# jgsimard/RustRobotics

Measured on AMD Instinct MI355X. Metric: GN iterations/s, higher is better.
Workload: dtype f64; 1 GPU; intel (1728 poses / 4830 edges / dim 5184), Gauss-Newton, one graph on one GPU; solver=GaussNewton, parallelism=single

## Files before the change

### rustrobotics_amd/csrc/kernels.hip.h

```cpp
#pragma once
#include <hip/hip_runtime.h>

#include <cstdint>
#include <type_traits>

#ifndef RRPGO_CHAIN_PRIO
#define RRPGO_CHAIN_PRIO 3
#endif

namespace rrpgo {

constexpr unsigned X_PENDING_WORD = 0x7ff8deadu;

template <typename T> struct VecT;
template <> struct VecT<float> { using V4 = float4; using V2 = float2; };
template <> struct VecT<double> { using V4 = double4; using V2 = double2; };

#ifndef RRPGO_LIN_GROUP
#define RRPGO_LIN_GROUP 8
#endif
constexpr int LIN_GROUP = RRPGO_LIN_GROUP;
constexpr int LIN_THREADS = 256;
constexpr int UPD_THREADS = 256;

// ... 41 lines not shown
#endif
#else
#define RRPGO_STAMP(a, s, slot) do { } while (0)
#define RRPGO_STAMP_SOLVE(a, s, slot) do { } while (0)
#define RRPGO_ACC_DECL() do { } while (0)
#define RRPGO_ACC_BEGIN() do { } while (0)
#define RRPGO_ACC_END(ptr, slot) do { } while (0)
#endif

__device__ __forceinline__ int wave_index() { return __builtin_amdgcn_readfirstlane((int)(threadIdx.x >> 6)); }

enum : int { DEVERR_NOT_SPD = 1, DEVERR_FLOW_TIMEOUT = 2 };

struct OptCtrl {
  double lambda;
  double last_error;
  double tolerance;
  unsigned long long seq;
  int reject;
  int pad;
};
struct alignas(32) OptSlot {
  double chi2, norm;
  int flags, pad;
  unsigned long long seq;
};
enum : int { OPT_RING = 8 };
enum : int { OPT_STOP = 1,
             OPT_SKIPPED = 2,
             OPT_ERR_SHIFT = 8
};
__device__ __forceinline__ void opt_publish(OptCtrl *c, OptSlot *ring, double chi2, double norm, int flags) {
  const unsigned long long n = c->seq + 1;
  OptSlot *s = ring + (n - 1) % OPT_RING;
  s->chi2 = chi2;
  s->norm = norm;
  s->flags = flags;
  __hip_atomic_store(&s->seq, n, __ATOMIC_RELEASE, __HIP_MEMORY_SCOPE_SYSTEM);
  c->seq = n;
}
__device__ __forceinline__ bool opt_stopped(const int *err) { return err && err[1] != 0; }


template <typename TC> struct EdgeRec {
  int32_t from, to;
  int64_t slot;
  typename VecT<TC>::V4 meas;
  typename VecT<TC>::V4 info_a;
  typename VecT<TC>::V2 info_b;
};
static_assert(sizeof(EdgeRec<float>) == 64 && sizeof(EdgeRec<double>) == 128, "EdgeRec is four / eight sixteen-byte loads of one line");
template <typename T, typename TC = T> struct LinArgs {
  int n_nodes;
  const EdgeRec<TC> *e_rec;
  const typename VecT<TC>::V4 *pose;
  const int2 *e_idx;
  const typename VecT<TC>::V4 *e_meas;
  const typename VecT<TC>::V4 *e_info_a;
  const typename VecT<TC>::V2 *e_info_b;
// ... 198 lines not shown

template <typename A> __device__ __forceinline__ void opt_publish_chi2_in_last_block(const A &a, double *red) {
  if (!a.publish) return;
  const bool stopped = !a.reset_ctrl && a.err[1] != 0;
  if (a.publish == 1 && !stopped) return;
  __shared__ int is_last;
  if (threadIdx.x == 0) {
    __threadfence();
    is_last = atomicAdd(a.blocks_done, 1) == (int)gridDim.x - 1;
  }
  __syncthreads();
  if (!is_last) return;
  __threadfence();
  double c = 0.0;
  for (int i = threadIdx.x; i < (int)gridDim.x; i += LIN_THREADS) c += a.chi2_partial[i];
  const double ct = block_sum<double, LIN_THREADS>(c, red);
  if (threadIdx.x == 0) {
    *a.blocks_done = 0;
    if (!stopped) a.ctrl->last_error = ct;
    opt_publish(a.ctrl, a.ring_host, ct, 0.0, stopped ? OPT_SKIPPED : 0);
  }
}

template <typename TO, typename T, int RK = ROBUST_NONE>
__global__ void __launch_bounds__(LIN_THREADS) k_linearize(LinArgs<TO, T> a) {
  using V4 = typename VecT<T>::V4;
  using V2 = typename VecT<T>::V2;
  __shared__ double red[LIN_THREADS / 64];
  const int gid = blockIdx.x * LIN_THREADS + threadIdx.x;
  for (int i = gid; i < a.n_zero_words; i += gridDim.x * LIN_THREADS) a.zero_words[i] = 0u;
  for (int i = gid; i < a.n_fill_words; i += gridDim.x * LIN_THREADS) a.fill_words[i] = X_PENDING_WORD;
  opt_reset_in_first_thread(a);
  const T lambda = a.lambda_from_ctrl ? (T)a.ctrl->lambda : a.lambda;
  const int slot = gid / LIN_GROUP, sub = gid % LIN_GROUP;
  const int node = slot < a.n_nodes ? (a.node_list ? a.node_list[slot] : slot) : -1;
  double chi = 0.0;
  T hd[6] = {0, 0, 0, 0, 0, 0};
  T bv[3] = {0, 0, 0};
  int nd = 0;
  if (node >= 0) {
    nd = a.node_dim[node];
    const V4 self = a.pose[node];
    const int q1 = a.inc_ptr[node + 1];
    for (int q = a.inc_ptr[node] + sub; q < q1; q += LIN_GROUP) {
      const int2 inc = a.inc_list[q];
      const int ent = inc.x;
      if (!(ent & 12)) continue;
      const bool owns = ent & 4;
      const int k = ent >> 4, kind = (ent >> 1) & 1, role = ent & 1;
      const EdgeRec<T> rec = a.e_rec[k];
      const V4 other = a.pose[inc.y];
      const V4 z = rec.meas;
      const V4 wa = rec.info_a;
      const V2 wb = rec.info_b;
      T W[3][3] = {{wa.x, wa.y, wa.z}, {wa.y, wa.w, wb.x}, {wa.z, wb.x, wb.y}};
      T e[3], A[3][3], B[3][3];
      edge_linearize_2d<T>(kind, role ? other : self, role ? self : other, z, e, A, B);
      T s_rob = 0;
      bool rob = false;
      if constexpr (RK != ROBUST_NONE) {
        s_rob = edge_chi2_2d<T>(W, e);
        rob = !a.robust_mask || a.robust_mask[k];
        if (rob) {
          const T w = robust_weight<RK, T>(s_rob, a.robust_delta, a.robust_delta2);
#pragma unroll
          for (int i = 0; i < 3; i++)
#pragma unroll
            for (int j = 0; j < 3; j++) W[i][j] *= w;
        }
      }
      T JW[3][3];
#pragma unroll
      for (int i = 0; i < 3; i++)
#pragma unroll
// ... 43 lines not shown
  if (a.write_system) {
#pragma unroll
    for (int t = 0; t < 6; t++) hd[t] = group_sum8(hd[t]);
#pragma unroll
    for (int t = 0; t < 3; t++) bv[t] = group_sum8(bv[t]);
    if (node >= 0 && sub == 0) {
      T add = lambda;
      if (node == a.anchor) add += (T)10000000.0;
      if (a.adds_diag && !a.adds_diag[node]) add = 0;
      TO *d = a.hvals + a.diag_off[node];
      if (nd == 3) {
        d[0] = (TO)(hd[0] + add); d[1] = (TO)hd[1];         d[2] = (TO)hd[3];
        d[3] = (TO)hd[1];         d[4] = (TO)(hd[2] + add); d[5] = (TO)hd[4];
        d[6] = (TO)hd[3];         d[7] = (TO)hd[4];         d[8] = (TO)(hd[5] + add);
      } else {
        d[0] = (TO)(hd[0] + add); d[1] = (TO)hd[1];
        d[2] = (TO)hd[1];         d[3] = (TO)(hd[2] + add);
      }
      TO *bo = a.b + a.node_offset[node];
      for (int t = 0; t < nd; t++) bo[t] = (TO)(-bv[t]);
    }
  }
  double tot = block_sum<double, LIN_THREADS>(chi, red);
  if (threadIdx.x == 0) a.chi2_partial[blockIdx.x] = tot;
  opt_publish_chi2_in_last_block(a, red);
}

template <typename TO, typename T>
__global__ void __launch_bounds__(256) k_lin_init(LinArgs<TO, T> a) {
  const int node = blockIdx.x * 256 + threadIdx.x;
  if (node >= a.n_nodes) return;
  const int nd = a.node_dim[node];
  T add = a.lambda;
  if (node == a.anchor) add += (T)10000000.0;
  TO *d = a.hvals + a.diag_off[node];
  for (int t = 0; t < nd * nd; t++) d[t] = (t / nd == t % nd) ? (TO)add : (TO)0;
  TO *bo = a.b + a.node_offset[node];
  for (int t = 0; t < nd; t++) bo[t] = 0;
}
template <typename TO, typename T>
__global__ void __launch_bounds__(256) k_lin_finish(LinArgs<TO, T> a) {
  const int node = blockIdx.x * 256 + threadIdx.x;
  if (node >= a.n_nodes) return;
  const int nd = a.node_dim[node];
  TO *d = a.hvals + a.diag_off[node];
  for (int i = 0; i < nd; i++)
    for (int j = i + 1; j < nd; j++) d[i * nd + j] = d[j * nd + i];
// ... 3005 lines not shown
  for (int i = j + threadIdx.x; i < a.nc; i += 256) col[i] += a0 * v0[i] + a1 * v1[i] + a2 * v2[i];
}


template <typename T, typename TC = T> struct UpdArgs {
  int n_nodes;
  typename VecT<TC>::V4 *pose;
  const uint8_t *node_dim;
  const int32_t *node_pcol, *node_offset;
  const T *x;
  const T *dx_ref_in;
  T *dx_ref_out;
  TC sign;
  double *norm_partial;
  int gauge_anchor;
  int export_only;
  const int *err;
  const int32_t *node_list;
  const uint8_t *norm_counts;
  const int *gate;
  FinArgs fin;
};

template <typename TO, typename T>
__device__ __forceinline__ double update_node(const UpdArgs<TO, T> &a, int node) {
  double nrm = 0.0;
  const int nd = a.node_dim[node];
  T d[3] = {0, 0, 0};
  const TO *src = a.dx_ref_in ? a.dx_ref_in + a.node_offset[node] : a.x + a.node_pcol[node];
  for (int t = 0; t < nd; t++) d[t] = (T)src[t];
  auto p = a.pose[node];
  const bool regauge = a.gauge_anchor >= 0 && !a.dx_ref_in;
  if (regauge) {
    const TO *ya = a.x + a.node_pcol[a.gauge_anchor];
    const T c0 = (T)ya[0], c1 = (T)ya[1], c2 = (T)ya[2];
    const auto pa = a.pose[a.gauge_anchor];
    d[0] = d[0] - c0 + c2 * (p.y - pa.y);
    d[1] = d[1] - c1 - c2 * (p.x - pa.x);
    if (nd == 3) d[2] -= c2;
    if (node == a.gauge_anchor) { d[0] = 0; d[1] = 0; d[2] = 0; }
  }
  if (a.dx_ref_out) {
    TO *dst = a.dx_ref_out + a.node_offset[node];
    for (int t = 0; t < nd; t++) dst[t] = (TO)d[t];
  }
  if (!a.export_only && !(regauge && node == a.gauge_anchor)) {
    if (!a.norm_counts || a.norm_counts[node])
      for (int t = 0; t < nd; t++) nrm += (double)d[t] * (double)d[t];
    p.x += a.sign * d[0];
    p.y += a.sign * d[1];
    if (nd == 3) {
      const T c = cos(a.sign * d[2]), s = sin(a.sign * d[2]);
      const T re = p.z * c - p.w * s, im = p.z * s + p.w * c;
      p.z = re;
      p.w = im;
    }
    a.pose[node] = p;
  }
  return nrm;
}

template <typename TO, typename T>
__global__ void __launch_bounds__(UPD_THREADS) k_update(UpdArgs<TO, T> a) {
  __shared__ double red[UPD_THREADS / 64];
  const int slot = blockIdx.x * UPD_THREADS + threadIdx.x;
  const int node = slot < a.n_nodes ? (a.node_list ? a.node_list[slot] : slot) : -1;
  double nrm = 0.0;
  if (a.gate && *a.gate == 0) return;
  const bool failed = a.err && (a.err[0] != 0 || a.err[1] != 0);
  if (node >= 0 && !failed) nrm = update_node(a, node);
  if (a.export_only) return;
  double tot = block_sum<double, UPD_THREADS>(nrm, red);
  if (threadIdx.x == 0) a.norm_partial[blockIdx.x] = tot;
  if (a.fin.enabled) finalize_in_last_block<UPD_THREADS>(a.fin, a.norm_partial, (int)gridDim.x, red);
}

}
```

### rustrobotics_amd/csrc/lds_flow.hip.h

```cpp
#pragma once

namespace rrpgo {

struct alignas(128) LdsFlowTask {
  SnMeta m;
  int32_t sn;
  int32_t sn_begin, sn_end;
  int32_t kind;
  int32_t slices;
  int32_t bx, by;
  int32_t n_units;
  int32_t pad[8];
};
static_assert(sizeof(LdsFlowTask) == 128, "LdsFlowTask is one 128-byte line");

__device__ __forceinline__ int lds_flow_ticket(unsigned *ticket, int *slot) {
  if (threadIdx.x == 0) *slot = (int)atomicAdd(ticket, 1u);
  __syncthreads();
  return __builtin_amdgcn_readfirstlane(*slot);
}

template <typename T, int THREADS>
__global__ void __launch_bounds__(THREADS) k_factor_flow(FactorArgs<T> a, const LdsFlowTask *tasks, int n_tasks, unsigned *ticket) {
  extern __shared__ __align__(16) unsigned char smem_raw[];
// ... 59 lines not shown
      __syncthreads();
      if (threadIdx.x == 0) __hip_atomic_fetch_add(a.dep_flags + a.parent_dep_self + tr.sn, 1u, __ATOMIC_RELAXED, __HIP_MEMORY_SCOPE_AGENT);
      continue;
    }
    if (tr.kind == 2) {
      dep_wait_count(a.dep_flags + a.parent_dep_self + tr.sn, (unsigned)tr.n_units, a.err, a.wait_ticks);
      solve_big_front<T, THREADS, true>(a, tr.m, smem, part, N, tr.slices);
      continue;
    }
    int snext = tr.sn;
    SnMeta mnext = tr.m;
    for (int si = tr.sn_end - 1; si >= tr.sn_begin; si--) {
      const int s = snext;
      const SnMeta m = mnext;
      if (si > tr.sn_begin) {
        snext = a.task_sn[si - 1];
        mnext = a.sn_meta[snext];
      }
      solve_front<T, THREADS, true, true>(a, s, m, smem);
    }
  }
}

__global__ void __launch_bounds__(256) k_fill_words(unsigned *w, int n, unsigned v) {
  for (int i = blockIdx.x * 256 + threadIdx.x; i < n; i += gridDim.x * 256) w[i] = v;
}

__global__ void __launch_bounds__(256) k_copy_words16(const uint4 *src, uint4 *dst, int64_t n) {
  for (int64_t i = (int64_t)blockIdx.x * 256 + threadIdx.x; i < n; i += (int64_t)gridDim.x * 256) dst[i] = src[i];
}

}
```

### rustrobotics_amd/csrc/pgo_api.hip

```cpp
#include <mutex>
#include <queue>
#include <hip/hip_runtime.h>

#include <algorithm>
#include <chrono>
#include <cmath>
#include <cstdio>
#include <cstdlib>
#include <cstring>
#include <functional>
#include <memory>
#include <stdexcept>
#include <string>
#include <thread>
#include <vector>

#include "../../include/rr_pgo.h"
#include "host_graph.h"
#include "kernels.hip.h"
#include "flow.hip.h"
#include "lds_flow.hip.h"
#include "selinv.hip.h"
#include "treesolve.hip.h"
#include "symbolic.h"
// ... 367 lines not shown
  static constexpr int kGemvSlices = 16;
  DevBuf<double> chi_partial_, norm_partial_, hist_;
  DevBuf<int> counter_, err_, blocks_done_;
  DevBuf<unsigned long long> stamps_;
  DevBuf<int32_t> task_ptr_, task_sn_, fasm_src_, fasm_dst_, fasm_colptr_, fdup_src_, fdup_dst_, scat_, rel_, perm_, sn_rows_;
  DevBuf<SnMeta> sn_meta_, task_meta_;
  DevBuf<ChildMeta> child_meta_;
  std::vector<int> step_solve_lds_;
  PinnedBuf<double> host_pair_;
  PinnedBuf<V4> state_stage_;
  EventHolder state_stage_ev_;
  std::vector<double> state_in_;
  DevBuf<V4> pose_saved_;
  OptSlot *opt_ring_ = nullptr;
  DevBuf<OptCtrl> opt_ctrl_;
  bool opt_active_ = false;
  bool opt_first_ = false;
  bool opt_lambda_dev_ = false;
  int opt_publish_ = 0;
  double opt_lambda0_ = 0.01;
  bool stop_dirty_ = false;
  bool sync_optimize_ = false;
  int n_lin_blocks_ = 0, n_upd_blocks_ = 0;
  bool no_graph_ = false, force_graph_ = false;
  bool edge_lin_ = false;
  bool edge_lin_wave_ = false;
  bool edge_lin_env_ = false, edge_lin_wave_env_ = false;
  int lin_blocks_pull_ = 0, lin_blocks_edge_ = 0;
  int robust_kind_ = ROBUST_NONE;
  double robust_delta_ = 1.0;
  DevBuf<uint8_t> robust_mask_;
  int host_counter_ = 0;

 public:
  Engine(const HostGraph &g, const Symbolic &sym, int rank, int world, bool sharded)
      : g_(g), sym_(sym), rank_(rank), world_(world), sharded_(sharded || world > 1) {
    struct ArenaScope {
      explicit ArenaScope(DeviceArena *a) { t_arena = a; }
      ~ArenaScope() { t_arena = nullptr; }
    } scope(&arena_);
    const bool ctimes = getenv("RR_PGO_ANALYZE_TIMES") != nullptr;
    double ct0 = now_ms();
    auto cmark = [&](const char *what) {
      if (!ctimes) return;
      const double t = now_ms();
      std::fprintf(stderr, "engine:  %-12s %8.3f ms\n", what, t - ct0);
// ... 137 lines not shown
      bool any_big = false;
      for (const Step &st : sym.steps) any_big = any_big || st.kind != STEP_TASKS;
      gemv_part_.alloc(any_big ? (size_t)kGemvSlices * g.dim : 4);
    }
    if (const char *e = getenv("RR_PGO_SOLVE_THREADS")) solve_threads_max_ = std::atoi(e);
    if (const char *e = getenv("RR_PGO_SP_SOLVE_MIN")) sp_solve_min_nc_ = std::atoi(e);
    if (const char *e = getenv("RR_PGO_SCHUR_SPLIT")) schur_split_ = std::atoi(e) != 0;
    no_graph_ = getenv("RR_PGO_NO_GRAPH") != nullptr;
    force_graph_ = getenv("RR_PGO_FORCE_GRAPH") != nullptr && !no_graph_;
    if (const char *e = getenv("RR_PGO_FLOW")) flow_max_nf_ = std::atoi(e);
    if (const char *e = getenv("RR_PGO_FLOW_EXACT")) flow_exact_ = std::atoi(e) != 0;
    if (const char *e = getenv("RR_PGO_FLOW_TASKS")) flow_max_tasks_ = std::atoi(e);
    if (const char *e = getenv("RR_PGO_SOLVE_FLOW")) solve_flow_on_ = std::atoi(e) != 0;
    if (const char *e = getenv("RR_PGO_FLOW_SCHUR_MIN")) flow_schur_min_ = std::atoi(e);
    n_lin_blocks_ = (int)(((int64_t)n_list_ * LIN_GROUP + LIN_THREADS - 1) / LIN_THREADS);
    lin_blocks_pull_ = n_lin_blocks_;
    edge_lin_ = getenv("RR_PGO_EDGE_LINEARIZE") != nullptr && !is3d_ && !sharded_ && g_.n_edges() > 0;
    edge_lin_wave_ = edge_lin_ && std::atoi(getenv("RR_PGO_EDGE_LINEARIZE")) == 2;
    if (edge_lin_) n_lin_blocks_ = std::max(1, (g_.n_edges() + (edge_lin_wave_ ? WE_EDGES : LIN_THREADS) - 1) / (edge_lin_wave_ ? WE_EDGES : LIN_THREADS));
    edge_lin_env_ = edge_lin_;
    edge_lin_wave_env_ = edge_lin_wave_;
    lin_blocks_edge_ = n_lin_blocks_;
    n_upd_blocks_ = (n_list_ + UPD_THREADS - 1) / UPD_THREADS;
    chi_partial_.alloc((size_t)(edge_lin_ ? std::max(lin_blocks_pull_, lin_blocks_edge_) : n_lin_blocks_));
    norm_partial_.alloc((size_t)n_upd_blocks_);
    hist_.alloc(2 * HIST);
    hist_.zero();
    counter_.alloc(1);
    counter_.zero();
    err_.alloc(2);
    err_.zero();
    opt_ctrl_.alloc(1);
    opt_ctrl_.zero();
    sync_optimize_ = getenv("RR_PGO_SYNC_OPTIMIZE") != nullptr;
    blocks_done_.alloc(2);
    blocks_done_.zero();
    cmark("numeric");
    task_ptr_.upload(sym.task_ptr);
    task_sn_.upload(sym.task_sn);
    {
      std::vector<SnMeta> meta(sym.S);
      std::vector<ChildMeta> cm(sym.child_list.size());
      int64_t wblk_total = 0;
      for (int f = 0; f < sym.S; f++) {
        SnMeta &m = meta[f];
        m.nc = sym.sn_ncols[f];
        m.nr = sym.sn_nrows[f];
// ... 151 lines not shown
        for (int t = st.task_begin; t < st.task_end; t++) {
          int s = sym.task_sn[sym.task_ptr[t]];
          need = std::max(need, sym.sn_ncols[s] + sym.sn_nrows[s] + 64 * 65 + 4);
        }
      }
      if ((size_t)need * sizeof(T) > (size_t)kMaxLds) throw ApiError(RR_PGO_EUNSUPPORTED, "front too large for the back-substitution scratch");
      step_solve_lds_.push_back(need);
    }
#ifdef RRPGO_STAMPS
    stamps_.alloc((size_t)sym.S * 12 + 400000);
    stamps_.zero();
#endif
    plan_mid_solve_tasks();
    cmark("index tables");
    configure_kernels();
    cmark("kernel attrs");
    n_launches_per_iter = 2;
    for (const Step &st : sym.steps)
      n_launches_per_iter += st.kind == STEP_BIG ? count_big_launches(st) + count_big_solve_launches(st) : 2;
    if (lds_flow_) {
      n_launches_per_iter = 4 + (xl_ ? 1 : 0);
      for (size_t si = 1; si < sym.steps.size(); si++)
        n_launches_per_iter += (xl_ ? 0 : count_big_launches(sym.steps[si])) + (mid_in_flow_[si] ? 0 : count_big_solve_launches(sym.steps[si]));
    }
  }

  ~Engine() override {
    if (gn_exec_) (void)hipGraphExecDestroy(gn_exec_);
    for (hipGraphExec_t e : stage_exec_) if (e) (void)hipGraphExecDestroy(e);
  }

  hipStream_t stream() override { return stream_; }

 private:
  void build_flow_levels() {
    flow_levels_.clear();
    flow_levels_.resize(sym_.steps.size());
    solve_flow_.clear();
    solve_flow_.resize(sym_.steps.size());
    constexpr double kDiag = 4.0, kPre = 2.5, kNewest = 1.5, kX = 1.5, kLook = 4.5, kTile = 8.0, kTail = 4.5, kHop = 0.7;
    int64_t words = 0;
    int dev = 0, cus = 256;
    HIPCHK(hipGetDevice(&dev));
    (void)hipDeviceGetAttribute(&cus, hipDeviceAttributeMultiprocessorCount, dev);
    flow_grid_ = std::max(cus, 1) * (sizeof(T) == 4 ? RRPGO_FLOW_WAVES : 1);
    if (const char *e = getenv("RR_PGO_FLOW_GRID")) flow_grid_ = std::max(1, std::atoi(e));
// ... 703 lines not shown
    int64_t n[RR_PGO_NUM_KCLASS] = {0};
  } prof_;
  void pbegin() { if (prof_.on) HIPCHK(hipEventRecord(prof_.e0, stream_)); }
  void pend(int k, int launches = 1) {
    if (!prof_.on) return;
    HIPCHK(hipEventRecord(prof_.e1, stream_));
    HIPCHK(hipEventSynchronize(prof_.e1));
    float ms = 0;
    HIPCHK(hipEventElapsedTime(&ms, prof_.e0, prof_.e1));
    prof_.ms[k] += ms;
    prof_.n[k] += launches;
  }

  void check_launch(const char *what) {
    hipError_t e = hipGetLastError();
    if (e != hipSuccess) throw ApiError(RR_PGO_ENODEVICE, std::string("kernel launch failed (") + what + "): " + hipGetErrorString(e));
  }

  void launch_linearize(double lambda, int lm, int write_system, bool reference_prior = false) {
    if (stop_dirty_ && !opt_active_) {
      HIPCHK(hipMemsetAsync(err_.p + 1, 0, sizeof(int), stream_));
      stop_dirty_ = false;
    }
    pbegin();
    if (!is3d_ && edge_lin_) {
      const LinArgs<T, S> la = lin_args(lambda, lm, write_system, reference_prior);
      const unsigned nb = (unsigned)((g_.n_nodes() + 255) / 256);
      if (lds_flow_) {
        hipLaunchKernelGGL(k_fill_words, dim3(4), dim3(256), 0, stream_, dep_flags_.p, 2 * sym_.S + 64, 0u);
        hipLaunchKernelGGL(k_fill_words, dim3(16), dim3(256), 0, stream_, reinterpret_cast<unsigned *>(x_ptr_), (int)((size_t)g_.dim * sizeof(T) / 4), X_PENDING_WORD);
      }
      if (write_system) hipLaunchKernelGGL((k_lin_init<T, S>), dim3(nb), dim3(256), 0, stream_, la);
      if (edge_lin_wave_) hipLaunchKernelGGL((k_linearize_wave_edges<T, S>), dim3(n_lin_blocks_), dim3(256), 0, stream_, la, g_.n_edges());
      else hipLaunchKernelGGL((k_linearize_edges<T, S>), dim3(n_lin_blocks_), dim3(LIN_THREADS), 0, stream_, la, g_.n_edges());
      if (write_system) hipLaunchKernelGGL((k_lin_finish<T, S>), dim3(nb), dim3(256), 0, stream_, la);
    } else if (!is3d_) {
      if (robust_kind_ == ROBUST_HUBER)
        hipLaunchKernelGGL((k_linearize<T, S, ROBUST_HUBER>), dim3(n_lin_blocks_), dim3(LIN_THREADS), 0, stream_,
                           lin_args(lambda, lm, write_system, reference_prior));
      else if (robust_kind_ == ROBUST_CAUCHY)
        hipLaunchKernelGGL((k_linearize<T, S, ROBUST_CAUCHY>), dim3(n_lin_blocks_), dim3(LIN_THREADS), 0, stream_,
                           lin_args(lambda, lm, write_system, reference_prior));
      else
        hipLaunchKernelGGL((k_linearize<T, S>), dim3(n_lin_blocks_), dim3(LIN_THREADS), 0, stream_,
                           lin_args(lambda, lm, write_system, reference_prior));
    } else {
// ... 248 lines not shown
            const SolveFlowLevel &sl = *solve_flow_[(size_t)i];
            int cus_grid = std::min(sl.n_tasks, std::max(flow_grid_ / (sizeof(T) == 4 ? RRPGO_FLOW_WAVES : 1), 1));
            hipLaunchKernelGGL(k_big_solve_flow<T>, dim3((unsigned)cus_grid), dim3(1024), 0, stream_, fa, (const T *)gemv_part_.p, (int64_t)g_.dim, R,
                               flow_flags_.p, (const SolveFlowFront *)sl.fronts.p, (const SolveFlowTask *)sl.tasks.p, sl.n_tasks,
                               flow_flags_.p + sl.ticket_word);
            check_launch("k_big_solve_flow");
            pend(RR_PGO_K_BIG_SOLVE, 2);
            continue;
          }
          const int nsp = (max_nc + BIG_SUPER - 1) / BIG_SUPER;
          for (int ell = 0; ell < nsp; ell++) {
            hipLaunchKernelGGL(k_big_solve_sp<T>, dim3(1 + (max_nc + 63) / 64, nf), dim3(1024), 0, stream_, fa, ell, (const T *)gemv_part_.p, (int64_t)g_.dim, R);
            check_launch("k_big_solve_sp");
          }
          pend(RR_PGO_K_BIG_SOLVE, 1 + nsp);
          continue;
        }
        hipLaunchKernelGGL((k_solve_mid<T, 1024>), dim3(nf), dim3(1024), lds, stream_, fa, 1, (const T *)gemv_part_.p, (int64_t)g_.dim, R);
        pend(RR_PGO_K_BIG_SOLVE, 2);
      }
    }
  }

  void launch_update(const T *dx_ref_in, double sign, bool write_ref, bool export_only = false, bool fused_finalize = false, const int *gate = nullptr) {
    FinArgs fin{};
    if (fused_finalize) {
      fin.enabled = 1; fin.chi_partial = chi_partial_.p; fin.n_chi = n_lin_blocks_; fin.hist = hist_.p; fin.counter = counter_.p;
      fin.advance = 1; fin.ring = HIST; fin.blocks_done = blocks_done_.p;
      if (opt_active_) { fin.ctrl = opt_ctrl_.p; fin.ring_host = opt_ring_; fin.err = err_.p; }
    }
    pbegin();
    if (!is3d_) {
      UpdArgs<T, S> u;
      u.n_nodes = n_list_;
      u.node_list = node_list_.p;
      u.norm_counts = norm_counts_.p;
      u.pose = pose_.p;
      u.node_dim = node_dim_.p;
      u.node_pcol = node_pcol_.p;
      u.node_offset = node_offset_.p;
      u.x = x_ptr_;
      u.dx_ref_in = dx_ref_in;
      u.dx_ref_out = write_ref ? dx_ref_.p : nullptr;
      u.sign = (S)sign;
      u.norm_partial = norm_partial_.p;
      u.gauge_anchor = (!dx_ref_in && gauge_now_) ? g_.anchor_node : -1;
      u.export_only = export_only ? 1 : 0;
      u.err = dx_ref_in ? nullptr : err_.p;
      u.gate = gate;
      u.fin = fin;
      hipLaunchKernelGGL((k_update<T, S>), dim3(n_upd_blocks_), dim3(UPD_THREADS), 0, stream_, u);
    } else {
      UpdArgs3<T, S> u;
      u.n_nodes = n_list_;
      u.node_list = node_list_.p;
      u.norm_counts = norm_counts_.p;
      u.pose = pose_.p;
      u.node_pcol = node_pcol_.p;
      u.node_offset = node_offset_.p;
      u.x = x_ptr_;
      u.dx_ref_in = dx_ref_in;
      u.dx_ref_out = write_ref ? dx_ref_.p : nullptr;
      u.sign = (S)sign;
      u.norm_partial = norm_partial_.p;
      u.export_only = export_only ? 1 : 0;
      u.err = dx_ref_in ? nullptr : err_.p;
      u.gate = gate;
      u.fin = fin;
      hipLaunchKernelGGL((k_update_se3<T, S>), dim3(n_upd_blocks_), dim3(UPD_THREADS), 0, stream_, u);
    }
    check_launch("k_update");
    pend(RR_PGO_K_UPDATE);
  }

  void launch_finalize(bool chi, bool norm, bool advance) {
    pbegin();
    hipLaunchKernelGGL(k_finalize_slot, dim3(1), dim3(256), 0, stream_, chi_partial_.p, chi ? n_lin_blocks_ : 0,
                       norm_partial_.p, norm ? n_upd_blocks_ : 0, hist_.p, counter_.p, advance ? 1 : 0);
    pend(RR_PGO_K_REDUCE);
  }

  void enqueue_gn_iteration() {
    launch_linearize(0.0, 0, 1);
    launch_factor();
    launch_solve();
    launch_update(nullptr, 1.0, true, false, true);
  }

  void ensure_gn_graph() {
    if (gn_exec_) return;
    hipGraph_t graph = nullptr;
    HIPCHK(hipStreamBeginCapture(stream_, hipStreamCaptureModeThreadLocal));
    try {
      enqueue_gn_iteration();
    } catch (...) {
      (void)hipStreamEndCapture(stream_, &graph);
      if (graph) (void)hipGraphDestroy(graph);
      throw;
    }
    HIPCHK(hipStreamEndCapture(stream_, &graph));
    const hipError_t ie = hipGraphInstantiate(&gn_exec_, graph, nullptr, nullptr, 0);
    (void)hipGraphDestroy(graph);
    if (ie != hipSuccess) { gn_exec_ = nullptr; throw ApiError(RR_PGO_ENODEVICE, std::string("hipGraphInstantiate: ") + hipGetErrorString(ie)); }
  }

  void read_slot(int slot, double *chi, double *norm) {
    int *eflag = reinterpret_cast<int *>(host_pair_.p + 2);
    HIPCHK(hipMemcpyAsync(host_pair_.p, hist_.p + 2 * (slot % HIST), 2 * sizeof(double), hipMemcpyDeviceToHost, stream_));
    HIPCHK(hipMemcpyAsync(eflag, err_.p, sizeof(int), hipMemcpyDeviceToHost, stream_));
    HIPCHK(hipStreamSynchronize(stream_));
    if (chi) *chi = host_pair_[0];
// ... 49 lines not shown
    HIPCHK(hipStreamSynchronize(stream_));
    check_device_error();
    for (int i = 0; i < g_.dim; i++) dx_out[i] = (double)tmp[i];
  }

  void update(const double *dx, double sign) override {
    refuse_rank_partial("rr_pgo_update");
    std::vector<T> tmp((size_t)g_.dim);
    for (int i = 0; i < g_.dim; i++) tmp[i] = (T)dx[i];
    HIPCHK(hipMemcpyAsync(dx_ref_.p, tmp.data(), tmp.size() * sizeof(T), hipMemcpyHostToDevice, stream_));
    launch_update(dx_ref_.p, sign, false);
    HIPCHK(hipStreamSynchronize(stream_));
  }

  void optimize(int solver, int iters, double *errors, int *n_errors, double *norms) override {
    if (sharded_) throw ApiError(RR_PGO_EUNSUPPORTED, "sharded handle: drive it with rr_pgo_stage + the two collectives");
    if (!edge_lin_ && !sync_optimize_ && !prof_.on && n_launches_per_iter < 48) {
      optimize_pipelined(solver, iters, errors, n_errors, norms);
      return;
    }
    const double tolerance = 1e-4;
    int ne = 0;
    if (solver == RR_PGO_GAUSS_NEWTON) {
      const bool eager = (no_graph_ || n_launches_per_iter <= 8) && !gn_exec_ && !force_graph_;
      if (!eager) ensure_gn_graph();
      reset_counter();
      int done = 0;
      for (int i = 0; i < iters; i++) {
        if (eager) enqueue_gn_iteration();
        else HIPCHK(hipGraphLaunch(gn_exec_, stream_));
        double chi, nrm;
        read_slot(i, &chi, &nrm);
        errors[ne++] = chi;
        if (norms) norms[i] = nrm;
        done = i + 1;
        if (nrm < tolerance) break;
      }
      (void)done;
      errors[ne++] = chi2_now();
    } else {
      double lambda = 0.01;
      double last_error = chi2_now();
      errors[ne++] = last_error;
      for (int i = 0; i < iters; i++) {
        reset_counter();
        launch_linearize(lambda, 1, 1);
        launch_factor();
// ... 5 lines not shown
        double error, nrm;
        read_slot(0, &error, &nrm);
        if (last_error < error) {
          launch_update(dx_ref_.p, -1.0, false);
          lambda *= 2.0;
        } else {
          lambda /= 2.0;
        }
        last_error = error;
        if (norms) norms[i] = nrm;
        errors[ne++] = error;
        if (nrm < tolerance) break;
      }
      HIPCHK(hipStreamSynchronize(stream_));
    }
    *n_errors = ne;
  }

  void enqueue_opt_item(bool lm, long k, int iters) {
    OptItemArgs oi{};
    oi.chi_partial = chi_partial_.p; oi.norm_partial = norm_partial_.p; oi.n_chi = n_lin_blocks_; oi.n_norm = 0; oi.mode = 0;
    oi.ctrl = opt_ctrl_.p; oi.ring = opt_ring_; oi.err = err_.p;
    struct Pub { int &p; ~Pub() { p = 0; } } pub{opt_publish_};
    if (!lm) {
      opt_publish_ = k < iters ? 1 : 2;
      if (k < iters) enqueue_gn_iteration();
      else launch_linearize(0.0, 0, 0);
      return;
    }
    if (k == 0) {
      launch_linearize(0.0, 0, 0);
      hipLaunchKernelGGL(k_opt_item, dim3(1), dim3(256), 0, stream_, oi);
      check_launch("k_opt_item");
      return;
    }
    launch_linearize(0.0, 1, 1);
    launch_factor();
    launch_solve();
    launch_update(nullptr, 1.0, true);
    launch_linearize(0.0, 0, 0);
    oi.n_norm = n_upd_blocks_; oi.mode = 1;
    hipLaunchKernelGGL(k_opt_item, dim3(1), dim3(256), 0, stream_, oi);
    check_launch("k_opt_item");
    launch_update(dx_ref_.p, -1.0, false, false, false, &opt_ctrl_.p->reject);
  }
  bool wait_opt_slot(long idx, OptSlot *out) {
    volatile OptSlot *s = opt_ring_ + idx % OPT_RING;
    const unsigned long long want = (unsigned long long)idx + 1;
    double t_query = now_ms();
    for (unsigned spins = 0;; spins++) {
      if (__atomic_load_n(const_cast<unsigned long long *>(&s->seq), __ATOMIC_ACQUIRE) == want) break;
      __builtin_ia32_pause();
      if ((spins & 1023u) == 1023u && now_ms() - t_query > 1.0) {
        const hipError_t q = hipStreamQuery(stream_);
        if (q == hipSuccess) {
          if (__atomic_load_n(const_cast<unsigned long long *>(&s->seq), __ATOMIC_ACQUIRE) == want) break;
          return false;
        }
        if (q != hipErrorNotReady) throw ApiError(RR_PGO_ENODEVICE, std::string("hipStreamQuery: ") + hipGetErrorString(q));
        t_query = now_ms();
      }
    }
    out->chi2 = s->chi2; out->norm = s->norm; out->flags = s->flags; out->seq = want;
    return true;
  }
  void optimize_pipelined(int solver, int iters, double *errors, int *n_errors, double *norms) {
    const bool lm = solver != RR_PGO_GAUSS_NEWTON;
    const long total = (long)iters + 1;
    for (int i = 0; i < OPT_RING; i++) opt_ring_[i].seq = 0ull;
    struct Scope {
      Engine *e;
      bool done = false;
      ~Scope() {
        e->opt_active_ = false; e->opt_first_ = false; e->stop_dirty_ = true;
        if (!done) (void)hipStreamSynchronize(e->stream_);
      }
    } scope{this};
    opt_active_ = true; opt_first_ = true; opt_lambda_dev_ = lm; opt_lambda0_ = 0.01;
    long enq = 0, seen = 0;
    int ne = 0, dev_err = 0;
    bool stop_seen = false;
    while (true) {
      while (enq < total && enq < seen + 2 && !stop_seen) enqueue_opt_item(lm, enq++, iters);
      if (seen >= enq) break;
      OptSlot sl;
      if (!wait_opt_slot(seen, &sl)) {
        HIPCHK(hipStreamSynchronize(stream_));
        check_device_error();
        throw ApiError(RR_PGO_ENODEVICE, "internal: an item of rr_pgo_optimize was never published");
      }
      const long k = seen++;
      const int e = sl.flags >> OPT_ERR_SHIFT;
      if (e) { dev_err = e; stop_seen = true; continue; }
      if (!lm) {
        if (k == iters || (sl.flags & OPT_SKIPPED)) { if (!dev_err) errors[ne++] = sl.chi2; continue; }
        errors[ne++] = sl.chi2;
        if (norms) norms[k] = sl.norm;
      } else {
        if (sl.flags & OPT_SKIPPED) continue;
        errors[ne++] = sl.chi2;
        if (k > 0 && norms) norms[k - 1] = sl.norm;
      }
      if (sl.flags & OPT_STOP) stop_seen = true;
    }
    scope.done = true;
    if (dev_err) throw_on_flag(dev_err);
    *n_errors = ne;
  }

  void get_state(double *out) override {
    const int N = g_.n_nodes();
    std::vector<V4> pose(pose_.n);
    HIPCHK(hipMemcpyAsync(pose.data(), pose_.p, pose.size() * sizeof(V4), hipMemcpyDeviceToHost, stream_));
    HIPCHK(hipStreamSynchronize(stream_));
    for (int i = 0; i < N; i++) {
      if (is3d_) {
        const V4 &t = pose[2 * i], &q = pose[2 * i + 1];
// ... 42 lines not shown
        pose[i] = V4{(S)st[0], (S)st[1], (S)0, (S)0};
        st += 2;
      }
    }
    HIPCHK(hipMemcpyAsync(pose_saved_.p, pose, pose_.n * sizeof(V4), hipMemcpyHostToDevice, stream_));
    HIPCHK(hipEventRecord(state_stage_ev_, stream_));
    restore_saved_state();
  }

  void assemble(double lambda, int lm, std::vector<double> &hv, std::vector<double> &b) override {
    refuse_rank_partial("rr_pgo_assemble");
    launch_linearize(lambda, lm, 1, true);
    std::vector<T> th((size_t)sym_.n_hvals), tb((size_t)g_.dim);
    HIPCHK(hipMemcpyAsync(th.data(), hvals_.p, th.size() * sizeof(T), hipMemcpyDeviceToHost, stream_));
    HIPCHK(hipMemcpyAsync(tb.data(), b_.p, tb.size() * sizeof(T), hipMemcpyDeviceToHost, stream_));
    HIPCHK(hipStreamSynchronize(stream_));
    hv.assign(th.begin(), th.end());
    b.assign(tb.begin(), tb.end());
  }

  void iterate_async(int iters) override {
    if (sharded_) throw ApiError(RR_PGO_EUNSUPPORTED, "sharded handle: drive it with rr_pgo_stage + the two collectives");
    if (no_graph_ || !force_graph_) {
      for (int i = 0; i < iters; i++) enqueue_gn_iteration();
      return;
    }
    ensure_gn_graph();
    for (int i = 0; i < iters; i++) HIPCHK(hipGraphLaunch(gn_exec_, stream_));
  }

  void sync() override {
    HIPCHK(hipStreamSynchronize(stream_));
    check_device_error();
  }

  int schur_tile() const override { return schur_split_ ? schur_tile_ : 0; }
  void solve_form(int32_t *kform, double *k_bytes, double *k_flops) const override {
    *kform = kform_ ? 1 : 0;
    if (k_bytes) *k_bytes = kform_bytes_;
    if (k_flops) *k_flops = kform_flops_;
  }
  void mark_flow_fronts(std::vector<char> &in_flow) override {
    for (size_t si = 0; si < flow_levels_.size(); si++)
      if (flow_levels_[si])
        for (int t = sym_.steps[si].task_begin; t < sym_.steps[si].task_end; t++)
          in_flow[sym_.task_sn[sym_.task_ptr[t]]] = flow_levels_[si]->schur_split ? 1 : 2;
// ... 1366 lines not shown
```

Baseline: 7595 GN iterations/s.

## Fuse pose update with next-iteration linearize in one ticketed kernel

Adds a k_update_linearize kernel that hands out update and linearize tasks by ticket. Linearize blocks spin-wait on a counter until every update block has written its poses, and poses go through buffer loads and stores. This removes one kernel launch per Gauss-Newton iteration and lets linearize blocks prefetch edge records while updates finish. Chi2 partials are double-buffered and the next chi2 is published in the ring slot, which changes how the host pipeline counts results. The cost is spin-wait synchronisation inside the kernel, plus a risk of deadlock if blocks are not all co-resident.

Result: no change. 7644 GN iterations/s, median of 6 (+0.7%).

```diff
diff --git a/rustrobotics_amd/csrc/kernels.hip.h b/rustrobotics_amd/csrc/kernels.hip.h
--- a/rustrobotics_amd/csrc/kernels.hip.h
+++ b/rustrobotics_amd/csrc/kernels.hip.h
@@ -87,6 +87,7 @@
 };
 struct alignas(32) OptSlot {
   double chi2, norm;
+  double chi2_next;
   int flags, pad;
   unsigned long long seq;
 };
@@ -95,11 +96,12 @@
              OPT_SKIPPED = 2,
              OPT_ERR_SHIFT = 8
 };
-__device__ __forceinline__ void opt_publish(OptCtrl *c, OptSlot *ring, double chi2, double norm, int flags) {
+__device__ __forceinline__ void opt_publish(OptCtrl *c, OptSlot *ring, double chi2, double norm, int flags, double chi2_next = 0.0) {
   const unsigned long long n = c->seq + 1;
   OptSlot *s = ring + (n - 1) % OPT_RING;
   s->chi2 = chi2;
   s->norm = norm;
+  s->chi2_next = chi2_next;
   s->flags = flags;
   __hip_atomic_store(&s->seq, n, __ATOMIC_RELEASE, __HIP_MEMORY_SCOPE_SYSTEM);
   c->seq = n;
@@ -344,34 +346,81 @@
   }
 }
 
-template <typename TO, typename T, int RK = ROBUST_NONE>
-__global__ void __launch_bounds__(LIN_THREADS) k_linearize(LinArgs<TO, T> a) {
+typedef unsigned rr_u4 __attribute__((ext_vector_type(4)));
+template <typename T, bool HANDOFF> struct PoseIo;
+template <typename T> struct PoseIo<T, false> {
+  using V4 = typename VecT<T>::V4;
+  V4 *p;
+  __device__ __forceinline__ PoseIo(const V4 *pose, int) : p(const_cast<V4 *>(pose)) {}
+  __device__ __forceinline__ V4 ld(int i) const { return p[i]; }
+  __device__ __forceinline__ void st(int i, const V4 &v) const { p[i] = v; }
+};
+template <typename T> struct PoseIo<T, true> {
+  using V4 = typename VecT<T>::V4;
+  static constexpr int kParts = (int)(sizeof(V4) / 16);
+  struct Words { rr_u4 w[kParts]; };
+  static_assert(sizeof(Words) == sizeof(V4), "a pose is one or two 16-byte words");
+  __amdgpu_buffer_rsrc_t r;
+  __device__ __forceinline__ PoseIo(const V4 *pose, int n)
+      : r(__builtin_amdgcn_make_buffer_rsrc(const_cast<V4 *>(pose), 0, n * (int)sizeof(V4), 0x00020000)) {}
+  __device__ __forceinline__ V4 ld(int i) const {
+    Words w;
+#pragma unroll
+    for (int k = 0; k < kParts; k++) w.w[k] = __builtin_amdgcn_raw_buffer_load_b128(r, i * (int)sizeof(V4) + 16 * k, 0, 16);
+    return __builtin_bit_cast(V4, w);
+  }
+  __device__ __forceinline__ void st(int i, const V4 &v) const {
+    const Words w = __builtin_bit_cast(Words, v);
+#pragma unroll
+    for (int k = 0; k < kParts; k++) __builtin_amdgcn_raw_buffer_store_b128(w.w[k], r, i * (int)sizeof(V4) + 16 * k, 0, 16);
+  }
+};
+__device__ __forceinline__ bool dep_wait_count(const unsigned *p, unsigned need, int *err, unsigned long long max_ticks);
+
+template <typename TO, typename T, int RK, bool FUSED>
+__device__ __forceinline__ void linearize_task(const LinArgs<TO, T> &a, int blk, int nblk, double *red, const unsigned *upd_count = nullptr,
+                                               unsigned n_upd = 0, unsigned long long wait_ticks = 0) {
   using V4 = typename VecT<T>::V4;
   using V2 = typename VecT<T>::V2;
-  __shared__ double red[LIN_THREADS / 64];
-  const int gid = blockIdx.x * LIN_THREADS + threadIdx.x;
-  for (int i = gid; i < a.n_zero_words; i += gridDim.x * LIN_THREADS) a.zero_words[i] = 0u;
-  for (int i = gid; i < a.n_fill_words; i += gridDim.x * LIN_THREADS) a.fill_words[i] = X_PENDING_WORD;
-  opt_reset_in_first_thread(a);
+  const PoseIo<T, FUSED> poses(a.pose, a.n_nodes);
+  const int gid = blk * LIN_THREADS + threadIdx.x;
+  for (int i = gid; i < a.n_zero_words; i += nblk * LIN_THREADS) a.zero_words[i] = 0u;
+  if constexpr (!FUSED)
+    for (int i = gid; i < a.n_fill_words; i += nblk * LIN_THREADS) a.fill_words[i] = X_PENDING_WORD;
   const T lambda = a.lambda_from_ctrl ? (T)a.ctrl->lambda : a.lambda;
   const int slot = gid / LIN_GROUP, sub = gid % LIN_GROUP;
   const int node = slot < a.n_nodes ? (a.node_list ? a.node_list[slot] : slot) : -1;
   double chi = 0.0;
   T hd[6] = {0, 0, 0, 0, 0, 0};
   T bv[3] = {0, 0, 0};
-  int nd = 0;
+  int nd = 0, q0 = 0, q1 = 0;
   if (node >= 0) {
     nd = a.node_dim[node];
-    const V4 self = a.pose[node];
-    const int q1 = a.inc_ptr[node + 1];
-    for (int q = a.inc_ptr[node] + sub; q < q1; q += LIN_GROUP) {
+    q0 = a.inc_ptr[node] + sub;
+    q1 = a.inc_ptr[node + 1];
+    if constexpr (FUSED)
+      if (q0 < q1) {
+        const EdgeRec<T> *rec = a.e_rec + (a.inc_list[q0].x >> 4);
+        const int32_t head = rec->from;
+        const T tail = rec->info_b.x;
+        asm volatile("" ::"v"(head), "v"(tail));
+      }
+  }
+  if constexpr (FUSED) {
+    if (threadIdx.x < 64) dep_wait_count(upd_count, n_upd, a.err, wait_ticks);
+    __syncthreads();
+    for (int i = gid; i < a.n_fill_words; i += nblk * LIN_THREADS) a.fill_words[i] = X_PENDING_WORD;
+  }
+  if (node >= 0) {
+    const V4 self = poses.ld(node);
+    for (int q = q0; q < q1; q += LIN_GROUP) {
       const int2 inc = a.inc_list[q];
       const int ent = inc.x;
       if (!(ent & 12)) continue;
       const bool owns = ent & 4;
       const int k = ent >> 4, kind = (ent >> 1) & 1, role = ent & 1;
       const EdgeRec<T> rec = a.e_rec[k];
-      const V4 other = a.pose[inc.y];
+      const V4 other = poses.ld(inc.y);
       const V4 z = rec.meas;
       const V4 wa = rec.info_a;
       const V2 wb = rec.info_b;
@@ -461,7 +510,20 @@
     }
   }
   double tot = block_sum<double, LIN_THREADS>(chi, red);
-  if (threadIdx.x == 0) a.chi2_partial[blockIdx.x] = tot;
+  if (threadIdx.x == 0) {
+    if constexpr (FUSED) {
+      __hip_atomic_store(a.chi2_partial + blk, tot, __ATOMIC_RELAXED, __HIP_MEMORY_SCOPE_AGENT);
+      asm volatile("s_waitcnt vmcnt(0)" ::: "memory");
+    } else {
+      a.chi2_partial[blk] = tot;
+    }
+  }
+}
+template <typename TO, typename T, int RK = ROBUST_NONE>
+__global__ void __launch_bounds__(LIN_THREADS) k_linearize(LinArgs<TO, T> a) {
+  __shared__ double red[LIN_THREADS / 64];
+  opt_reset_in_first_thread(a);
+  linearize_task<TO, T, RK, false>(a, (int)blockIdx.x, (int)gridDim.x, red);
   opt_publish_chi2_in_last_block(a, red);
 }
 
@@ -3513,7 +3575,7 @@
   FinArgs fin;
 };
 
-template <typename TO, typename T>
+template <typename TO, typename T, bool HANDOFF = false>
 __device__ __forceinline__ double update_node(const UpdArgs<TO, T> &a, int node) {
   double nrm = 0.0;
   const int nd = a.node_dim[node];
@@ -3546,7 +3608,7 @@
       p.z = re;
       p.w = im;
     }
-    a.pose[node] = p;
+    PoseIo<T, HANDOFF>(a.pose, a.n_nodes).st(node, p);
   }
   return nrm;
 }
diff --git a/rustrobotics_amd/csrc/lds_flow.hip.h b/rustrobotics_amd/csrc/lds_flow.hip.h
--- a/rustrobotics_amd/csrc/lds_flow.hip.h
+++ b/rustrobotics_amd/csrc/lds_flow.hip.h
@@ -105,6 +105,69 @@
   }
 }
 
+template <typename T, typename TC = T> struct UpdLinArgs {
+  UpdArgs<T, TC> u;
+  LinArgs<T, TC> l;
+  int n_upd, n_lin;
+  unsigned *words;
+  const double *chi_prev;
+  unsigned long long wait_ticks;
+};
+template <typename TO, typename T, int RK = ROBUST_NONE>
+__global__ void __launch_bounds__(LIN_THREADS) k_update_linearize(UpdLinArgs<TO, T> a) {
+  static_assert(LIN_THREADS == UPD_THREADS, "one workgroup shape for both kinds of task");
+  __shared__ double red[LIN_THREADS / 64];
+  __shared__ int ticket_slot[2];
+  __shared__ int is_last;
+  if (opt_stopped(a.l.err)) return;
+  const int n_tasks = a.n_upd + a.n_lin;
+  const bool one_each = (int)gridDim.x >= n_tasks;
+  for (int round = 0;; round++) {
+    const int tk = lds_flow_ticket(a.words, &ticket_slot[round & 1]);
+    if (tk >= n_tasks) break;
+    if (tk < a.n_upd) {
+      const int slot = tk * UPD_THREADS + threadIdx.x;
+      const int node = slot < a.u.n_nodes ? (a.u.node_list ? a.u.node_list[slot] : slot) : -1;
+      const bool failed = a.u.err[0] != 0;
+      double nrm = 0.0;
+      if (node >= 0 && !failed) nrm = update_node<TO, T, true>(a.u, node);
+      dep_drain();
+      const double tot = block_sum<double, UPD_THREADS>(nrm, red);
+      if (threadIdx.x == 0) {
+        __hip_atomic_fetch_add(a.words + 32, 1u, __ATOMIC_RELAXED, __HIP_MEMORY_SCOPE_AGENT);
+        __hip_atomic_store(a.u.norm_partial + tk, tot, __ATOMIC_RELAXED, __HIP_MEMORY_SCOPE_AGENT);
+        asm volatile("s_waitcnt vmcnt(0)" ::: "memory");
+      }
+    } else {
+      linearize_task<TO, T, RK, true>(a.l, tk - a.n_upd, a.n_lin, red, a.words + 32, (unsigned)a.n_upd, a.wait_ticks);
+    }
+    if (one_each) break;
+  }
+  if (threadIdx.x == 0) is_last = __hip_atomic_fetch_add(a.words + 64, 1u, __ATOMIC_RELAXED, __HIP_MEMORY_SCOPE_AGENT) == gridDim.x - 1;
+  __syncthreads();
+  if (!is_last) return;
+  const FinArgs &f = a.u.fin;
+  double c = 0.0, n = 0.0, cn = 0.0;
+  for (int i = threadIdx.x; i < f.n_chi; i += LIN_THREADS) c += a.chi_prev[i];
+  for (int i = threadIdx.x; i < a.n_upd; i += LIN_THREADS) n += mem_ld<true>(a.u.norm_partial + i);
+  for (int i = threadIdx.x; i < a.n_lin; i += LIN_THREADS) cn += mem_ld<true>(a.l.chi2_partial + i);
+  const double ct = block_sum<double, LIN_THREADS>(c, red);
+  const double nt = block_sum<double, LIN_THREADS>(n, red);
+  const double cnt = block_sum<double, LIN_THREADS>(cn, red);
+  if (threadIdx.x != 0) return;
+  a.words[0] = 0u; a.words[32] = 0u; a.words[64] = 0u;
+  const int slot = *f.counter % f.ring;
+  f.hist[2 * slot] = ct;
+  f.hist[2 * slot + 1] = sqrt(nt);
+  if (f.advance) *f.counter = *f.counter + 1;
+  if (!f.ctrl) return;
+  const int e = __hip_atomic_load(f.err, __ATOMIC_RELAXED, __HIP_MEMORY_SCOPE_AGENT);
+  const double nrm = sqrt(nt);
+  const bool stop = e != 0 || nrm < f.ctrl->tolerance;
+  if (stop) f.err[1] = 1;
+  opt_publish(f.ctrl, f.ring_host, ct, nrm, (stop && !e ? OPT_STOP : 0) | (e << OPT_ERR_SHIFT), cnt);
+}
+
 __global__ void __launch_bounds__(256) k_fill_words(unsigned *w, int n, unsigned v) {
   for (int i = blockIdx.x * 256 + threadIdx.x; i < n; i += gridDim.x * 256) w[i] = v;
 }
diff --git a/rustrobotics_amd/csrc/pgo_api.hip b/rustrobotics_amd/csrc/pgo_api.hip
--- a/rustrobotics_amd/csrc/pgo_api.hip
+++ b/rustrobotics_amd/csrc/pgo_api.hip
@@ -413,6 +413,12 @@
   bool stop_dirty_ = false;
   bool sync_optimize_ = false;
   int n_lin_blocks_ = 0, n_upd_blocks_ = 0;
+  bool fuse_update_ = false;
+  int fused_saving_ = 0;
+  int fuse_grid_ = 0;
+  DevBuf<unsigned> ul_words_;
+  size_t chi_stride_ = 0;
+  int chi_cur_ = 0;
   bool no_graph_ = false, force_graph_ = false;
   bool edge_lin_ = false;
   bool edge_lin_wave_ = false;
@@ -596,7 +602,8 @@
     edge_lin_wave_env_ = edge_lin_wave_;
     lin_blocks_edge_ = n_lin_blocks_;
     n_upd_blocks_ = (n_list_ + UPD_THREADS - 1) / UPD_THREADS;
-    chi_partial_.alloc((size_t)(edge_lin_ ? std::max(lin_blocks_pull_, lin_blocks_edge_) : n_lin_blocks_));
+    chi_stride_ = (size_t)(edge_lin_ ? std::max(lin_blocks_pull_, lin_blocks_edge_) : n_lin_blocks_);
+    chi_partial_.alloc(2 * chi_stride_);
     norm_partial_.alloc((size_t)n_upd_blocks_);
     hist_.alloc(2 * HIST);
     hist_.zero();
@@ -794,6 +801,14 @@
       n_launches_per_iter = 4 + (xl_ ? 1 : 0);
       for (size_t si = 1; si < sym.steps.size(); si++)
         n_launches_per_iter += (xl_ ? 0 : count_big_launches(sym.steps[si])) + (mid_in_flow_[si] ? 0 : count_big_solve_launches(sym.steps[si]));
+    }
+    fuse_update_ = !is3d_ && !sharded_ && world_ <= 1 && sizeof(S) == 8 && n_launches_per_iter < 48 && pose_.n * sizeof(V4) < ((size_t)1 << 31);
+    if (const char *e = getenv("RR_PGO_FUSE_UPDATE")) fuse_update_ = fuse_update_ && std::atoi(e) != 0;
+    if (const char *e = getenv("RR_PGO_LDS_FLOW_GRID")) fuse_grid_ = std::max(1, std::atoi(e));
+    if (fuse_update_) {
+      ul_words_.alloc(96);
+      ul_words_.zero();
+      if (fused_form()) { n_launches_per_iter -= 1; fused_saving_ = 1; }
     }
   }
 
@@ -1543,6 +1558,7 @@
       HIPCHK(hipMemsetAsync(err_.p + 1, 0, sizeof(int), stream_));
       stop_dirty_ = false;
     }
+    chi_cur_ = 0;
     pbegin();
     if (!is3d_ && edge_lin_) {
       const LinArgs<T, S> la = lin_args(lambda, lm, write_system, reference_prior);
@@ -1837,34 +1853,39 @@
     }
   }
 
+  FinArgs fin_args() {
+    FinArgs fin{};
+    fin.enabled = 1; fin.chi_partial = chi_partial_.p + chi_cur_ * chi_stride_; fin.n_chi = n_lin_blocks_; fin.hist = hist_.p; fin.counter = counter_.p;
+    fin.advance = 1; fin.ring = HIST; fin.blocks_done = blocks_done_.p;
+    if (opt_active_) { fin.ctrl = opt_ctrl_.p; fin.ring_host = opt_ring_; fin.err = err_.p; }
+    return fin;
+  }
+  UpdArgs<T, S> upd_args(const T *dx_ref_in, double sign, bool write_ref, bool export_only, const int *gate, const FinArgs &fin) {
+    UpdArgs<T, S> u;
+    u.n_nodes = n_list_;
+    u.node_list = node_list_.p;
+    u.norm_counts = norm_counts_.p;
+    u.pose = pose_.p;
+    u.node_dim = node_dim_.p;
+    u.node_pcol = node_pcol_.p;
+    u.node_offset = node_offset_.p;
+    u.x = x_ptr_;
+    u.dx_ref_in = dx_ref_in;
+    u.dx_ref_out = write_ref ? dx_ref_.p : nullptr;
+    u.sign = (S)sign;
+    u.norm_partial = norm_partial_.p;
+    u.gauge_anchor = (!dx_ref_in && gauge_now_) ? g_.anchor_node : -1;
+    u.export_only = export_only ? 1 : 0;
+    u.err = dx_ref_in ? nullptr : err_.p;
+    u.gate = gate;
+    u.fin = fin;
+    return u;
+  }
   void launch_update(const T *dx_ref_in, double sign, bool write_ref, bool export_only = false, bool fused_finalize = false, const int *gate = nullptr) {
-    FinArgs fin{};
-    if (fused_finalize) {
-      fin.enabled = 1; fin.chi_partial = chi_partial_.p; fin.n_chi = n_lin_blocks_; fin.hist = hist_.p; fin.counter = counter_.p;
-      fin.advance = 1; fin.ring = HIST; fin.blocks_done = blocks_done_.p;
-      if (opt_active_) { fin.ctrl = opt_ctrl_.p; fin.ring_host = opt_ring_; fin.err = err_.p; }
-    }
+    const FinArgs fin = fused_finalize ? fin_args() : FinArgs{};
     pbegin();
     if (!is3d_) {
-      UpdArgs<T, S> u;
-      u.n_nodes = n_list_;
-      u.node_list = node_list_.p;
-      u.norm_counts = norm_counts_.p;
-      u.pose = pose_.p;
-      u.node_dim = node_dim_.p;
-      u.node_pcol = node_pcol_.p;
-      u.node_offset = node_offset_.p;
-      u.x = x_ptr_;
-      u.dx_ref_in = dx_ref_in;
-      u.dx_ref_out = write_ref ? dx_ref_.p : nullptr;
-      u.sign = (S)sign;
-      u.norm_partial = norm_partial_.p;
-      u.gauge_anchor = (!dx_ref_in && gauge_now_) ? g_.anchor_node : -1;
-      u.export_only = export_only ? 1 : 0;
-      u.err = dx_ref_in ? nullptr : err_.p;
-      u.gate = gate;
-      u.fin = fin;
-      hipLaunchKernelGGL((k_update<T, S>), dim3(n_upd_blocks_), dim3(UPD_THREADS), 0, stream_, u);
+      hipLaunchKernelGGL((k_update<T, S>), dim3(n_upd_blocks_), dim3(UPD_THREADS), 0, stream_, upd_args(dx_ref_in, sign, write_ref, export_only, gate, fin));
     } else {
       UpdArgs3<T, S> u;
       u.n_nodes = n_list_;
@@ -1902,6 +1923,32 @@
     launch_update(nullptr, 1.0, true, false, true);
   }
 
+  bool fused_form() const { return fuse_update_ && !edge_lin_ && !sync_optimize_ && !prof_.on; }
+  void launch_update_linearize(int write_system) {
+    UpdLinArgs<T, S> a;
+    a.u = upd_args(nullptr, 1.0, true, false, nullptr, fin_args());
+    a.l = lin_args(0.0, 0, write_system);
+    a.chi_prev = chi_partial_.p + chi_cur_ * chi_stride_;
+    chi_cur_ ^= 1;
+    a.l.chi2_partial = chi_partial_.p + chi_cur_ * chi_stride_;
+    a.n_upd = n_upd_blocks_;
+    a.n_lin = n_lin_blocks_;
+    a.words = ul_words_.p;
+    a.wait_ticks = wait_ticks_;
+    const int n_tasks = a.n_upd + a.n_lin;
+    const dim3 grid((unsigned)(fuse_grid_ > 0 ? std::min(fuse_grid_, n_tasks) : n_tasks));
+    if (robust_kind_ == ROBUST_HUBER) hipLaunchKernelGGL((k_update_linearize<T, S, ROBUST_HUBER>), grid, dim3(LIN_THREADS), 0, stream_, a);
+    else if (robust_kind_ == ROBUST_CAUCHY) hipLaunchKernelGGL((k_update_linearize<T, S, ROBUST_CAUCHY>), grid, dim3(LIN_THREADS), 0, stream_, a);
+    else hipLaunchKernelGGL((k_update_linearize<T, S>), grid, dim3(LIN_THREADS), 0, stream_, a);
+    check_launch("k_update_linearize");
+  }
+  void enqueue_gn_iteration_fused(long k) {
+    if (k == 0) launch_linearize(0.0, 0, 1);
+    else launch_update_linearize(1);
+    launch_factor();
+    launch_solve();
+  }
+
   void ensure_gn_graph() {
     if (gn_exec_) return;
     hipGraph_t graph = nullptr;
@@ -1997,7 +2044,7 @@
     const double tolerance = 1e-4;
     int ne = 0;
     if (solver == RR_PGO_GAUSS_NEWTON) {
-      const bool eager = (no_graph_ || n_launches_per_iter <= 8) && !gn_exec_ && !force_graph_;
+      const bool eager = (no_graph_ || n_launches_per_iter + fused_saving_ <= 8) && !gn_exec_ && !force_graph_;
       if (!eager) ensure_gn_graph();
       reset_counter();
       int done = 0;
@@ -2049,6 +2096,11 @@
     oi.chi_partial = chi_partial_.p; oi.norm_partial = norm_partial_.p; oi.n_chi = n_lin_blocks_; oi.n_norm = 0; oi.mode = 0;
     oi.ctrl = opt_ctrl_.p; oi.ring = opt_ring_; oi.err = err_.p;
     struct Pub { int &p; ~Pub() { p = 0; } } pub{opt_publish_};
+    if (!lm && iters > 0 && fused_form()) {
+      if (k < iters) enqueue_gn_iteration_fused(k);
+      else launch_update_linearize(0);
+      return;
+    }
     if (!lm) {
       opt_publish_ = k < iters ? 1 : 2;
       if (k < iters) enqueue_gn_iteration();
@@ -2088,7 +2140,7 @@
         t_query = now_ms();
       }
     }
-    out->chi2 = s->chi2; out->norm = s->norm; out->flags = s->flags; out->seq = want;
+    out->chi2 = s->chi2; out->norm = s->norm; out->chi2_next = s->chi2_next; out->flags = s->flags; out->seq = want;
     return true;
   }
   void optimize_pipelined(int solver, int iters, double *errors, int *n_errors, double *norms) {
@@ -2104,12 +2156,13 @@
       }
     } scope{this};
     opt_active_ = true; opt_first_ = true; opt_lambda_dev_ = lm; opt_lambda0_ = 0.01;
+    const bool fused = !lm && iters > 0 && fused_form();
     long enq = 0, seen = 0;
     int ne = 0, dev_err = 0;
     bool stop_seen = false;
     while (true) {
       while (enq < total && enq < seen + 2 && !stop_seen) enqueue_opt_item(lm, enq++, iters);
-      if (seen >= enq) break;
+      if (seen >= (fused ? enq - 1 : enq)) break;
       OptSlot sl;
       if (!wait_opt_slot(seen, &sl)) {
         HIPCHK(hipStreamSynchronize(stream_));
@@ -2119,7 +2172,11 @@
       const long k = seen++;
       const int e = sl.flags >> OPT_ERR_SHIFT;
       if (e) { dev_err = e; stop_seen = true; continue; }
-      if (!lm) {
+      if (fused) {
+        errors[ne++] = sl.chi2;
+        if (norms) norms[k] = sl.norm;
+        if ((sl.flags & OPT_STOP) || k == iters - 1) errors[ne++] = sl.chi2_next;
+      } else if (!lm) {
         if (k == iters || (sl.flags & OPT_SKIPPED)) { if (!dev_err) errors[ne++] = sl.chi2; continue; }
         errors[ne++] = sl.chi2;
         if (norms) norms[k] = sl.norm;
@@ -2208,6 +2265,11 @@
   void iterate_async(int iters) override {
     if (sharded_) throw ApiError(RR_PGO_EUNSUPPORTED, "sharded handle: drive it with rr_pgo_stage + the two collectives");
     if (no_graph_ || !force_graph_) {
+      if (fused_form() && iters > 0) {
+        for (int i = 0; i < iters; i++) enqueue_gn_iteration_fused(i);
+        launch_update(nullptr, 1.0, true, false, true);
+        return;
+      }
       for (int i = 0; i < iters; i++) enqueue_gn_iteration();
       return;
     }
```
